# sebrahimi1988/dss-ml-at-scale

Measured on AMD Instinct MI355X. Metric: samples/sec, higher is better.
Workload: dtype bf16; 1 GPU; model=resnet18, global_batch=212, parallelism=dp1+hipgraph

## Files before the change

mi355x_scale/ops/csrc/bindings.cpp:

```cpp

#include <torch/extension.h>
#include <ATen/hip/HIPContext.h>
#include <hip/hip_runtime.h>

extern "C" void launch_normalize_u8_to_bf16(
    const uint8_t* in, void* out, const float* scale_dev,
    const float* shift_dev, long long n, hipStream_t stream);

void normalize_u8_to_bf16(torch::Tensor in, torch::Tensor out,
                          torch::Tensor scale, torch::Tensor shift) {
  TORCH_CHECK(in.is_cuda() && out.is_cuda(), "tensors must be on GPU");
  TORCH_CHECK(in.scalar_type() == torch::kUInt8, "input must be uint8");
  TORCH_CHECK(out.scalar_type() == torch::kBFloat16, "output must be bf16");
  TORCH_CHECK(in.is_contiguous(), "input must be contiguous (NHWC)");
  TORCH_CHECK(in.numel() == out.numel(), "element count mismatch");
  TORCH_CHECK(scale.is_cuda() && shift.is_cuda() && scale.numel() == 3 &&
                  shift.numel() == 3,
              "scale/shift must be 3-element device float tensors");
  TORCH_CHECK(scale.scalar_type() == torch::kFloat32 &&
              shift.scalar_type() == torch::kFloat32,
              "scale/shift must be float32");
  auto stream = at::cuda::getCurrentHIPStream();
  launch_normalize_u8_to_bf16(
      in.data_ptr<uint8_t>(), out.data_ptr(),
// ... 107 lines not shown
}

void diff_center(torch::Tensor yT, torch::Tensor wc, torch::Tensor wm,
                 int64_t S, int64_t d) {
  _check_f32(yT, "yT"); _check_f32(wc, "wc"); _check_f32(wm, "wm");
  auto stream = at::cuda::getCurrentHIPStream();
  launch_diff_center(yT.data_ptr<float>(), wc.data_ptr<float>(),
                     wm.data_ptr<float>(), yT.size(0), yT.size(1),
                     (int)S, (int)d, stream.stream());
}

void exog_project_mfma(torch::Tensor P, torch::Tensor wc,
                       torch::Tensor beta) {
  _check_f32(P, "P"); _check_f32(wc, "wc"); _check_f32(beta, "beta");
  TORCH_CHECK(P.size(1) == wc.size(0), "K mismatch");
  TORCH_CHECK(beta.size(0) == P.size(0) && beta.size(1) == wc.size(1));
  TORCH_CHECK(P.size(0) <= 16, "KX must fit one MFMA row tile");
  auto stream = at::cuda::getCurrentHIPStream();
  launch_exog_project_mfma(P.data_ptr<float>(), wc.data_ptr<float>(),
                           beta.data_ptr<float>(), P.size(1), wc.size(1),
                           P.size(0), stream.stream());
}


extern "C" int bn_reduce_blocks(long long rows, int C);
extern "C" void launch_bn_fwd_reduce(const void* x, float* partial,
                                     int nblocks, long long rows, int C,
                                     hipStream_t stream);
extern "C" void launch_bn_fwd_finalize(const float* partial, int nblocks,
                                       float* mean, float* invstd,
                                       float* running_mean,
                                       float* running_var, float momentum,
                                       float eps, long long rows, int C,
                                       int update_running, hipStream_t stream);
extern "C" void launch_bn_fwd_apply(const void* x, const void* res, void* y,
                                    const float* mean, const float* invstd,
                                    const float* weight, const float* bias,
                                    long long rows, int C, int relu,
                                    hipStream_t stream);
extern "C" void launch_bn_bwd_reduce(const void* dz, const void* y,
                                     const void* x, const float* mean,
                                     const float* invstd, float* partial,
                                     void* dym, int nblocks, long long rows,
                                     int C, int relu, hipStream_t stream);
extern "C" void launch_bn_bwd_reduce_rm(const void* dz, const void* x,
                                        const float* mean,
                                        const float* invstd,
                                        const float* weight,
                                        const float* bias, float* partial,
                                        void* dym, int nblocks,
                                        long long rows, int C,
                                        hipStream_t stream);
extern "C" void launch_bn_bwd_apply_rm(const void* dz, const void* x,
                                       const float* mean,
                                       const float* invstd,
                                       const float* bias, const float* k,
                                       void* dx, long long rows, int C,
                                       hipStream_t stream);
extern "C" void launch_bn_bwd_apply_dym(const void* dym, const void* x,
                                        const float* mean,
                                        const float* invstd, const float* k,
                                        void* dx, long long rows, int C,
                                        hipStream_t stream);
extern "C" void launch_bn_bwd_finalize(const float* partial, int nblocks,
                                       const float* invstd,
                                       const float* weight, float* dweight,
                                       float* dbias, float* k, long long rows,
// ... 2 lines not shown
extern "C" void launch_bn_bwd_apply(const void* dz, const void* y,
                                    const void* x, const float* mean,
                                    const float* invstd, const float* k,
                                    void* dx, void* dres, long long rows,
                                    int C, int relu, hipStream_t stream);

static void _check_bn_act(const torch::Tensor& t, const char* name) {
  TORCH_CHECK(t.is_cuda() && t.scalar_type() == torch::kBFloat16,
              name, " must be bf16 on GPU");
}

static long long _bn_rows(const torch::Tensor& x, int64_t C) {
  TORCH_CHECK(C % 8 == 0 && 256 % (C / 8) == 0,
              "C must be 8*2^k and <= 2048, got ", C);
  TORCH_CHECK(x.numel() % C == 0, "numel not divisible by C");
  return (long long)(x.numel() / C);
}

torch::Tensor bn_fwd_reduce(torch::Tensor x, int64_t C) {
  _check_bn_act(x, "x");
  long long rows = _bn_rows(x, C);
  int nb = bn_reduce_blocks(rows, (int)C);
  auto partial = torch::empty(
      {(int64_t)nb * 2 * C},
      torch::TensorOptions().dtype(torch::kFloat32).device(x.device()));
  launch_bn_fwd_reduce(x.data_ptr(), partial.data_ptr<float>(), nb, rows,
                       (int)C, at::cuda::getCurrentHIPStream().stream());
  return partial;
}

void bn_fwd_finalize(torch::Tensor partial, torch::Tensor mean,
                     torch::Tensor invstd, torch::Tensor running_mean,
                     torch::Tensor running_var, double momentum, double eps,
                     int64_t rows, int64_t C, bool update_running) {
  _check_f32(partial, "partial"); _check_f32(mean, "mean");
  _check_f32(invstd, "invstd");
  _check_f32(running_mean, "running_mean");
  _check_f32(running_var, "running_var");
  TORCH_CHECK(partial.numel() % (2 * C) == 0, "partial must be [nb*2C]");
  int nb = (int)(partial.numel() / (2 * C));
  launch_bn_fwd_finalize(partial.data_ptr<float>(), nb,
                         mean.data_ptr<float>(), invstd.data_ptr<float>(),
                         running_mean.data_ptr<float>(),
                         running_var.data_ptr<float>(), (float)momentum,
                         (float)eps, rows, (int)C, update_running ? 1 : 0,
                         at::cuda::getCurrentHIPStream().stream());
}

void bn_fwd_apply(torch::Tensor x, torch::Tensor res, torch::Tensor y,
                  torch::Tensor mean, torch::Tensor invstd,
                  torch::Tensor weight, torch::Tensor bias, int64_t C,
                  bool relu) {
  _check_bn_act(x, "x"); _check_bn_act(y, "y");
  _check_f32(mean, "mean"); _check_f32(invstd, "invstd");
  _check_f32(weight, "weight"); _check_f32(bias, "bias");
  const void* res_p = nullptr;
  if (res.defined() && res.numel()) {
    _check_bn_act(res, "res");
    TORCH_CHECK(res.numel() == x.numel(), "residual shape mismatch");
    res_p = res.data_ptr();
  }
  launch_bn_fwd_apply(x.data_ptr(), res_p, y.data_ptr(),
                      mean.data_ptr<float>(), invstd.data_ptr<float>(),
                      weight.data_ptr<float>(), bias.data_ptr<float>(),
                      _bn_rows(x, C), (int)C, relu ? 1 : 0,
                      at::cuda::getCurrentHIPStream().stream());
}

torch::Tensor bn_bwd_reduce(torch::Tensor dz, torch::Tensor y,
                            torch::Tensor x, torch::Tensor mean,
                            torch::Tensor invstd, torch::Tensor dym,
                            int64_t C, bool relu) {
  _check_bn_act(dz, "dz"); _check_bn_act(y, "y"); _check_bn_act(x, "x");
  void* dym_p = nullptr;
  if (dym.defined() && dym.numel()) {
    _check_bn_act(dym, "dym");
    TORCH_CHECK(dym.numel() == x.numel(), "dym shape mismatch");
    dym_p = dym.data_ptr();
  }
// ... 154 lines not shown
}

void bn_maxpool3x3s2_fwd(torch::Tensor x, torch::Tensor mean,
                         torch::Tensor invstd, torch::Tensor weight,
                         torch::Tensor bias, torch::Tensor y,
                         torch::Tensor code) {
  _check_bn_act(x, "x"); _check_bn_act(y, "y");
  _check_f32(mean, "mean"); _check_f32(invstd, "invstd");
  _check_f32(weight, "weight"); _check_f32(bias, "bias");
  TORCH_CHECK(code.scalar_type() == torch::kUInt8 && code.is_cuda());
  int N = x.size(0), C = x.size(1), H = x.size(2), W = x.size(3);
  int Ho = y.size(2), Wo = y.size(3);
  TORCH_CHECK(C % 8 == 0 && 256 % (C / 8) == 0, "bad C");
  TORCH_CHECK(Ho == (H + 1) / 2 && Wo == (W + 1) / 2, "3x3 s2 p1 shape");
  TORCH_CHECK(code.numel() == y.numel());
  launch_bn_maxpool_fwd(x.data_ptr(), mean.data_ptr<float>(),
                        invstd.data_ptr<float>(),
                        weight.data_ptr<float>(), bias.data_ptr<float>(),
                        y.data_ptr(), code.data_ptr<uint8_t>(),
                        N, H, W, Ho, Wo, C,
                        at::cuda::getCurrentHIPStream().stream());
}

void maxpool3x3s2_bwd(torch::Tensor dy, torch::Tensor code,
                      torch::Tensor dx) {
  _check_bn_act(dy, "dy"); _check_bn_act(dx, "dx");
  TORCH_CHECK(code.scalar_type() == torch::kUInt8 && code.is_cuda());
  int N = dx.size(0), C = dx.size(1), H = dx.size(2), W = dx.size(3);
  int Ho = dy.size(2), Wo = dy.size(3);
  TORCH_CHECK(code.numel() == dy.numel());
  launch_maxpool_bwd(dy.data_ptr(), code.data_ptr<uint8_t>(),
                     dx.data_ptr(), N, H, W, Ho, Wo, C,
                     at::cuda::getCurrentHIPStream().stream());
}

extern "C" void launch_adam_step(float* p, const float* g, float* m,
                                 float* v, int* step, float lr, float beta1,
                                 float beta2, float eps, float weight_decay,
                                 long long n, hipStream_t stream);

void adam_step(torch::Tensor p, torch::Tensor g, torch::Tensor m,
               torch::Tensor v, torch::Tensor step, double lr, double beta1,
               double beta2, double eps, double weight_decay) {
  _check_f32(p, "p"); _check_f32(g, "g"); _check_f32(m, "m");
  _check_f32(v, "v");
  TORCH_CHECK(step.is_cuda() && step.scalar_type() == torch::kInt32 &&
                  step.numel() == 1,
              "step must be a 1-element int32 device tensor");
  long long n = p.numel();
  TORCH_CHECK(g.numel() == n && m.numel() == n && v.numel() == n,
              "flat buffer length mismatch");
  launch_adam_step(p.data_ptr<float>(), g.data_ptr<float>(),
                   m.data_ptr<float>(), v.data_ptr<float>(),
                   step.data_ptr<int>(), (float)lr, (float)beta1,
                   (float)beta2, (float)eps, (float)weight_decay, n,
                   at::cuda::getCurrentHIPStream().stream());
}

extern "C" void launch_adam_step_mixed(float* master, const void* gb,
                                       const float* gf, float* m, float* v,
                                       void* pb, int* step, float lr,
                                       float beta1, float beta2, float eps,
                                       float weight_decay, long long nb,
                                       long long n, hipStream_t stream);

void adam_step_mixed(torch::Tensor master, torch::Tensor gb,
// ... 79 lines not shown

int64_t conv3x3_wrw_nchunks(int64_t Nb, int64_t H, int64_t C,
                            int64_t chunks) {
  return conv3x3_wrw_chunks((int)Nb, (int)H, (int)C, (int)chunks);
}

PYBIND11_MODULE(TORCH_EXTENSION_NAME, m) {
  m.def("conv3x3_wrw", &conv3x3_wrw,
        "MFMA 3x3/s1 CxC weight grad (fp32 accum, bf16 cast to view)",
        pybind11::arg("x"), pybind11::arg("dy"), pybind11::arg("part"),
        pybind11::arg("dw"), pybind11::arg("phase_mask") = 7,
        pybind11::arg("chunks") = 0);
  m.def("conv3x3_wrw_nchunks", &conv3x3_wrw_nchunks,
        "partial-buffer chunk count the wrw launcher will use");
  m.def("stem_conv_fwd", &stem_conv_fwd,
        "MFMA stem conv fwd (7x7 s2, 3->64, NHWC bf16)",
        pybind11::arg("x"), pybind11::arg("w"), pybind11::arg("out"),
        pybind11::arg("wp_scratch"), pybind11::arg("phase_mask") = 7);
  m.def("stem_conv_wrw", &stem_conv_wrw,
        "MFMA stem conv weight-grad (fp32 accum + bf16 cast)",
        pybind11::arg("x"), pybind11::arg("dy"), pybind11::arg("dw_f32"),
        pybind11::arg("dw"), pybind11::arg("phase_mask") = 7);
  m.def("normalize_u8_to_bf16", &normalize_u8_to_bf16,
        "fused uint8 NHWC -> normalized bf16 (same memory order)");
  m.def("groupfit_eval", &groupfit_eval,
        "batched per-group ARIMAX candidate evaluation (validation MSE)");
  m.def("groupfit_final", &groupfit_final,
        "batched per-group final fit (fitted values + params)");
  m.def("diff_center", &diff_center,
        "difference + per-group centering of the time-major panel");
  m.def("exog_project_mfma", &exog_project_mfma,
        "design-matrix GEMM beta = P @ Wc on f32 MFMA");
  m.def("bn_fwd_reduce", &bn_fwd_reduce);
  m.def("bn_fwd_finalize", &bn_fwd_finalize);
  m.def("bn_fwd_apply", &bn_fwd_apply);
  m.def("bn_bwd_reduce", &bn_bwd_reduce);
  m.def("bn_bwd_reduce_rm", &bn_bwd_reduce_rm);
  m.def("bn_bwd_apply_rm", &bn_bwd_apply_rm);
  m.def("bn_bwd_finalize", &bn_bwd_finalize);
  m.def("bn_bwd_apply", &bn_bwd_apply);
  m.def("bn_bwd_apply_dym", &bn_bwd_apply_dym);
  m.def("adam_step", &adam_step,
        "fused flat Adam step (one kernel over p/g/m/v)");
  m.def("maxpool3x3s2_fwd", &maxpool3x3s2_fwd);
  m.def("bn_maxpool3x3s2_fwd", &bn_maxpool3x3s2_fwd);
  m.def("maxpool3x3s2_bwd", &maxpool3x3s2_bwd);
  m.def("adam_step_mixed", &adam_step_mixed,
        "fused flat Adam with bf16 params/grads + fp32 master");
  m.def("arma_generate", &arma_generate,
        "batched ARMA(p,q) sample paths, one group per lane");
}
```

mi355x_scale/ops/csrc/fused_bn.hip:

```cpp

#include <hip/hip_runtime.h>
#include <hip/hip_bf16.h>

typedef __hip_bfloat16 bf16;

#define VEC 8

union BVec {
  uint4 u;
  bf16 h[VEC];
};

static __device__ __forceinline__ BVec load8(const bf16* p) {
  BVec v;
  v.u = *reinterpret_cast<const uint4*>(p);
  return v;
}

static __device__ __forceinline__ void store8(bf16* p, const BVec& v) {
  *reinterpret_cast<uint4*>(p) = v.u;
}

__global__ __launch_bounds__(256) void bn_fwd_reduce_kernel(
    const bf16* __restrict__ x, float* __restrict__ partial,
// ... 16 lines not shown
    }
  }

  __shared__ float lds[256 * 2 * VEC];
  float* mys = &lds[(rsub * lanes + lane) * 2 * VEC];
#pragma unroll
  for (int j = 0; j < VEC; ++j) {
    mys[j] = s[j];
    mys[VEC + j] = q[j];
  }
  __syncthreads();
  for (int step = rows_per_iter >> 1; step > 0; step >>= 1) {
    if (rsub < step) {
      const float* other = &lds[((rsub + step) * lanes + lane) * 2 * VEC];
#pragma unroll
      for (int j = 0; j < 2 * VEC; ++j) mys[j] += other[j];
    }
    __syncthreads();
  }
  if (rsub == 0) {
#pragma unroll
    for (int j = 0; j < VEC; ++j) {
      partial[(long long)(lane * VEC + j) * gridDim.x + blockIdx.x] = mys[j];
      partial[(long long)(C + lane * VEC + j) * gridDim.x + blockIdx.x] =
          mys[VEC + j];
    }
  }
}

__global__ __launch_bounds__(256) void bn_fwd_finalize_kernel(
    const float* __restrict__ partial, int nblocks,
    float* __restrict__ mean, float* __restrict__ invstd,
    float* __restrict__ running_mean, float* __restrict__ running_var,
    float momentum, float eps, long long rows, int C, int update_running) {
  int c = blockIdx.x * (blockDim.x / 64) + threadIdx.x / 64;
  int lane = threadIdx.x % 64;
  if (c >= C) return;
  float s = 0.f, q = 0.f;
  for (int b = lane; b < nblocks; b += 64) {
    s += partial[(long long)c * nblocks + b];
    q += partial[(long long)(C + c) * nblocks + b];
  }
#pragma unroll
  for (int off = 32; off > 0; off >>= 1) {
    s += __shfl_down(s, off, 64);
    q += __shfl_down(q, off, 64);
  }
  if (lane != 0) return;
  float n = (float)rows;
  float m = s / n;
  float var = fmaxf(q / n - m * m, 0.f);
  mean[c] = m;
  invstd[c] = rsqrtf(var + eps);
  if (update_running) {
    float unbiased = rows > 1 ? var * (n / (n - 1.f)) : var;
    running_mean[c] = (1.f - momentum) * running_mean[c] + momentum * m;
    running_var[c] = (1.f - momentum) * running_var[c] + momentum * unbiased;
  }
}

template <bool RELU, bool RES>
__global__ __launch_bounds__(256) void bn_fwd_apply_kernel(
    const bf16* __restrict__ x, const bf16* __restrict__ res,
    bf16* __restrict__ y, const float* __restrict__ mean,
    const float* __restrict__ invstd, const float* __restrict__ weight,
    const float* __restrict__ bias, long long rows, int C) {
  const int lanes = C / VEC;
  const int lane = threadIdx.x % lanes;
  const int rsub = threadIdx.x / lanes;
  const int rows_per_iter = blockDim.x / lanes;
  const long long rstride = (long long)gridDim.x * rows_per_iter;

  float a[VEC], b[VEC];
#pragma unroll
  for (int j = 0; j < VEC; ++j) {
    int c = lane * VEC + j;
    a[j] = weight[c] * invstd[c];
    b[j] = bias[c] - mean[c] * a[j];
  }

  for (long long row = (long long)blockIdx.x * rows_per_iter + rsub;
       row < rows; row += rstride) {
    const long long off = row * C + (long long)lane * VEC;
    BVec v = load8(x + off);
    BVec r;
    if (RES) r = load8(res + off);
    BVec o;
#pragma unroll
    for (int j = 0; j < VEC; ++j) {
      float f = fmaf(__bfloat162float(v.h[j]), a[j], b[j]);
      if (RES) f += __bfloat162float(r.h[j]);
// ... 150 lines not shown
  float m[VEC], is[VEC], wv[VEC], k1[VEC], k2[VEC];
#pragma unroll
  for (int j = 0; j < VEC; ++j) {
    int c = lane * VEC + j;
    m[j] = mean[c];
    is[j] = invstd[c];
    wv[j] = k[c];
    k1[j] = k[C + c];
    k2[j] = k[2 * C + c];
  }

  for (long long row = (long long)blockIdx.x * rows_per_iter + rsub;
       row < rows; row += rstride) {
    const long long off = row * C + (long long)lane * VEC;
    BVec g = load8(dz + off);
    BVec xv = load8(x + off);
    BVec yv;
    if (RELU) yv = load8(y + off);
    BVec odx, odr;
#pragma unroll
    for (int j = 0; j < VEC; ++j) {
      float dy = __bfloat162float(g.h[j]);
      if (RELU && __bfloat162float(yv.h[j]) <= 0.f) dy = 0.f;
      float xhat = (__bfloat162float(xv.h[j]) - m[j]) * is[j];
      float v = wv[j] * (dy - k1[j] - xhat * k2[j]);
      odx.h[j] = __float2bfloat16(v);
      if (RES) odr.h[j] = __float2bfloat16(dy);
    }
    store8(dx + off, odx);
    if (RES) store8(dres + off, odr);
  }
}

template <bool WRITE_DY>
__global__ __launch_bounds__(256) void bn_bwd_reduce_rm_kernel(
    const bf16* __restrict__ dz, const bf16* __restrict__ x,
    const float* __restrict__ mean, const float* __restrict__ invstd,
    const float* __restrict__ weight, const float* __restrict__ bias,
    float* __restrict__ partial, bf16* __restrict__ dym,
    long long rows, int C) {
  const int lanes = C / VEC;
  const int lane = threadIdx.x % lanes;
  const int rsub = threadIdx.x / lanes;
  const int rows_per_iter = blockDim.x / lanes;
  const long long rstride = (long long)gridDim.x * rows_per_iter;

  float m[VEC], is[VEC], wv[VEC], bv[VEC];
#pragma unroll
  for (int j = 0; j < VEC; ++j) {
    int c = lane * VEC + j;
    m[j] = mean[c];
    is[j] = invstd[c];
    wv[j] = weight[c];
    bv[j] = bias[c];
  }

  float sdy[VEC] = {0.f}, sdyx[VEC] = {0.f};
  for (long long row = (long long)blockIdx.x * rows_per_iter + rsub;
       row < rows; row += rstride) {
    const long long off = row * C + (long long)lane * VEC;
    BVec g = load8(dz + off);
    BVec xv = load8(x + off);
    BVec dyv;
#pragma unroll
    for (int j = 0; j < VEC; ++j) {
      float xhat = (__bfloat162float(xv.h[j]) - m[j]) * is[j];
      float dy = __bfloat162float(g.h[j]);
      if (wv[j] * xhat + bv[j] <= 0.f) dy = 0.f;
      sdy[j] += dy;
      sdyx[j] += dy * xhat;
      if (WRITE_DY) dyv.h[j] = __float2bfloat16(dy);
    }
    if (WRITE_DY) store8(dym + off, dyv);
  }

  __shared__ float lds[256 * 2 * VEC];
  float* mys = &lds[(rsub * lanes + lane) * 2 * VEC];
#pragma unroll
  for (int j = 0; j < VEC; ++j) {
    mys[j] = sdy[j];
    mys[VEC + j] = sdyx[j];
  }
  __syncthreads();
  for (int step = rows_per_iter >> 1; step > 0; step >>= 1) {
    if (rsub < step) {
      const float* other = &lds[((rsub + step) * lanes + lane) * 2 * VEC];
#pragma unroll
      for (int j = 0; j < 2 * VEC; ++j) mys[j] += other[j];
    }
    __syncthreads();
  }
  if (rsub == 0) {
#pragma unroll
    for (int j = 0; j < VEC; ++j) {
      partial[(long long)(lane * VEC + j) * gridDim.x + blockIdx.x] = mys[j];
      partial[(long long)(C + lane * VEC + j) * gridDim.x + blockIdx.x] =
          mys[VEC + j];
    }
  }
}

__global__ __launch_bounds__(256) void bn_bwd_apply_rm_kernel(
    const bf16* __restrict__ dz, const bf16* __restrict__ x,
    const float* __restrict__ mean, const float* __restrict__ invstd,
    const float* __restrict__ bias, const float* __restrict__ k,
    bf16* __restrict__ dx, long long rows, int C) {
  const int lanes = C / VEC;
  const int lane = threadIdx.x % lanes;
  const int rsub = threadIdx.x / lanes;
  const int rows_per_iter = blockDim.x / lanes;
  const long long rstride = (long long)gridDim.x * rows_per_iter;

  float m[VEC], is[VEC], wis[VEC], k1[VEC], k2[VEC], bv[VEC], wv[VEC];
#pragma unroll
  for (int j = 0; j < VEC; ++j) {
    int c = lane * VEC + j;
    m[j] = mean[c];
    is[j] = invstd[c];
    wis[j] = k[c];
    k1[j] = k[C + c];
    k2[j] = k[2 * C + c];
    bv[j] = bias[c];
    wv[j] = wis[j] / is[j];
  }

  for (long long row = (long long)blockIdx.x * rows_per_iter + rsub;
       row < rows; row += rstride) {
    const long long off = row * C + (long long)lane * VEC;
    BVec g = load8(dz + off);
    BVec xv = load8(x + off);
    BVec odx;
#pragma unroll
    for (int j = 0; j < VEC; ++j) {
      float xhat = (__bfloat162float(xv.h[j]) - m[j]) * is[j];
      float dy = __bfloat162float(g.h[j]);
      if (wv[j] * xhat + bv[j] <= 0.f) dy = 0.f;
      float v = wis[j] * (dy - k1[j] - xhat * k2[j]);
      odx.h[j] = __float2bfloat16(v);
    }
    store8(dx + off, odx);
  }
}


static int pick_grid(long long rows, int C) {
  int rows_per_iter = 256 / (C / VEC);
  long long blocks = (rows + rows_per_iter - 1) / rows_per_iter;
  if (blocks > 2080) blocks = 2080;
  return (int)(blocks > 0 ? blocks : 1);
}

extern "C" int bn_reduce_blocks(long long rows, int C) {
  int rows_per_iter = 256 / (C / VEC);
  long long blocks = (rows + rows_per_iter - 1) / rows_per_iter;
  if (blocks > 512) blocks = 512;
  return (int)(blocks > 0 ? blocks : 1);
}

extern "C" void launch_bn_fwd_reduce(const void* x, float* partial,
                                     int nblocks, long long rows, int C,
                                     hipStream_t stream) {
  hipLaunchKernelGGL(bn_fwd_reduce_kernel, dim3(nblocks), dim3(256), 0,
                     stream, (const bf16*)x, partial, rows, C);
}

extern "C" void launch_bn_fwd_finalize(const float* partial, int nblocks,
                                       float* mean, float* invstd,
                                       float* running_mean,
                                       float* running_var, float momentum,
                                       float eps, long long rows, int C,
                                       int update_running,
                                       hipStream_t stream) {
  hipLaunchKernelGGL(bn_fwd_finalize_kernel, dim3((C + 3) / 4),
                     dim3(256), 0, stream, partial, nblocks, mean, invstd,
                     running_mean, running_var, momentum, eps, rows, C,
                     update_running);
}

extern "C" void launch_bn_fwd_apply(const void* x, const void* res, void* y,
                                    const float* mean, const float* invstd,
                                    const float* weight, const float* bias,
                                    long long rows, int C, int relu,
                                    hipStream_t stream) {
  dim3 grid(pick_grid(rows, C)), block(256);
#define APPLY(R, S)                                                       \
  hipLaunchKernelGGL((bn_fwd_apply_kernel<R, S>), grid, block, 0, stream, \
                     (const bf16*)x, (const bf16*)res, (bf16*)y, mean,    \
                     invstd, weight, bias, rows, C)
  if (relu && res) APPLY(true, true);
  else if (relu) APPLY(true, false);
  else if (res) APPLY(false, true);
  else APPLY(false, false);
#undef APPLY
}

extern "C" void launch_bn_bwd_reduce(const void* dz, const void* y,
                                     const void* x, const float* mean,
                                     const float* invstd, float* partial,
                                     void* dym, int nblocks, long long rows,
                                     int C, int relu, hipStream_t stream) {
  dim3 grid(nblocks), block(256);
#define REDUCE(R, W)                                                       \
  hipLaunchKernelGGL((bn_bwd_reduce_kernel<R, W>), grid, block, 0, stream, \
                     (const bf16*)dz, (const bf16*)y, (const bf16*)x,      \
                     mean, invstd, partial, (bf16*)dym, rows, C)
  if (relu && dym) REDUCE(true, true);
  else if (relu) REDUCE(true, false);
  else if (dym) REDUCE(false, true);
  else REDUCE(false, false);
// ... 1 lines not shown
}

extern "C" void launch_bn_bwd_reduce_rm(const void* dz, const void* x,
                                        const float* mean,
                                        const float* invstd,
                                        const float* weight,
                                        const float* bias, float* partial,
                                        void* dym, int nblocks,
                                        long long rows, int C,
                                        hipStream_t stream) {
  dim3 grid(nblocks), block(256);
  if (dym)
    hipLaunchKernelGGL((bn_bwd_reduce_rm_kernel<true>), grid, block, 0,
                       stream, (const bf16*)dz, (const bf16*)x, mean,
                       invstd, weight, bias, partial, (bf16*)dym, rows, C);
  else
    hipLaunchKernelGGL((bn_bwd_reduce_rm_kernel<false>), grid, block, 0,
                       stream, (const bf16*)dz, (const bf16*)x, mean,
                       invstd, weight, bias, partial, nullptr, rows, C);
}

extern "C" void launch_bn_bwd_apply_rm(const void* dz, const void* x,
                                       const float* mean,
                                       const float* invstd,
                                       const float* bias, const float* k,
                                       void* dx, long long rows, int C,
                                       hipStream_t stream) {
  hipLaunchKernelGGL(bn_bwd_apply_rm_kernel, dim3(pick_grid(rows, C)),
                     dim3(256), 0, stream, (const bf16*)dz,
                     (const bf16*)x, mean, invstd, bias, k, (bf16*)dx,
                     rows, C);
}

extern "C" void launch_bn_bwd_apply_dym(const void* dym, const void* x,
                                        const float* mean,
                                        const float* invstd, const float* k,
                                        void* dx, long long rows, int C,
                                        hipStream_t stream) {
  hipLaunchKernelGGL(bn_bwd_apply_dym_kernel, dim3(pick_grid(rows, C)),
                     dim3(256), 0, stream, (const bf16*)dym, (const bf16*)x,
                     mean, invstd, k, (bf16*)dx, rows, C);
}

extern "C" void launch_bn_bwd_finalize(const float* partial, int nblocks,
                                       const float* invstd,
                                       const float* weight, float* dweight,
                                       float* dbias, float* k, long long rows,
                                       int C, int accumulate,
                                       hipStream_t stream) {
  hipLaunchKernelGGL(bn_bwd_finalize_kernel, dim3((C + 3) / 4),
                     dim3(256), 0, stream, partial, nblocks, invstd, weight,
                     dweight, dbias, k, rows, C, accumulate);
}

extern "C" void launch_bn_bwd_apply(const void* dz, const void* y,
                                    const void* x, const float* mean,
                                    const float* invstd, const float* k,
                                    void* dx, void* dres, long long rows,
                                    int C, int relu, hipStream_t stream) {
  dim3 grid(pick_grid(rows, C)), block(256);
#define APPLY(R, S)                                                        \
  hipLaunchKernelGGL((bn_bwd_apply_kernel<R, S>), grid, block, 0, stream,  \
                     (const bf16*)dz, (const bf16*)y, (const bf16*)x,      \
                     mean, invstd, k, (bf16*)dx, (bf16*)dres, rows, C)
  if (relu && dres) APPLY(true, true);
  else if (relu) APPLY(true, false);
// ... 5 lines not shown
```

mi355x_scale/ops/fused_bn.py:

```python
from __future__ import annotations

from typing import Optional

import torch
import torch.nn as nn
import torch.nn.functional as F

from . import _C, require_ext


def _hip_supported(x: torch.Tensor) -> bool:
    c = x.shape[1]
    return (x.is_cuda and x.dtype == torch.bfloat16 and x.dim() == 4
            and c % 8 == 0 and c <= 2048 and (256 % (c // 8)) == 0)


class _FusedBNFn(torch.autograd.Function):
    @staticmethod
    def forward(ctx, x, residual, weight, bias, running_mean, running_var,
                momentum, eps, relu):
        C = x.shape[1]
        rows = x.numel() // C
        dev = x.device
        mean = torch.empty(C, dtype=torch.float32, device=dev)
        invstd = torch.empty(C, dtype=torch.float32, device=dev)
        partial = _C.bn_fwd_reduce(x, C)
        _C.bn_fwd_finalize(partial, mean, invstd, running_mean, running_var,
                           momentum, eps, rows, C, True)
        y = torch.empty_like(x)
        res = residual if residual is not None else x.new_empty(0)
        _C.bn_fwd_apply(x, res, y, mean, invstd, weight, bias, C, relu)
        ctx.save_for_backward(x, y if residual is not None else x,
                              mean, invstd, weight, bias)
        ctx.relu = relu
        ctx.has_res = residual is not None
        return y

    @staticmethod
    def backward(ctx, dz):
        x, y, mean, invstd, weight, bias = ctx.saved_tensors
        C = x.shape[1]
        rows = x.numel() // C
        dev = x.device
        if not dz.is_contiguous(memory_format=torch.channels_last):
            dz = dz.contiguous(memory_format=torch.channels_last)
        k = torch.empty(3 * C, dtype=torch.float32, device=dev)
        def _grad_view(p):
            g = p.grad
            if (g is not None and g.is_cuda and g.is_contiguous()
                    and g.dtype == torch.float32 and g.numel() == C):
                return g
            return None

        import os
        wg, bg = _grad_view(weight), _grad_view(bias)
        fuse_acc = (torch.cuda.is_current_stream_capturing()
                    and wg is not None and bg is not None
                    and os.environ.get("MI355X_BN_FUSED_ACC", "1") == "1")
        if fuse_acc:
            dweight, dbias = wg, bg
        else:
            dweight = torch.empty(C, dtype=torch.float32, device=dev)
            dbias = torch.empty(C, dtype=torch.float32, device=dev)
        dx = torch.empty_like(x)
        if ctx.has_res:
            dym = torch.empty_like(x)
            partial = _C.bn_bwd_reduce(dz, y, x, mean, invstd, dym, C,
                                       ctx.relu)
            _C.bn_bwd_finalize(partial, invstd, weight, dweight, dbias, k,
                               rows, C, fuse_acc)
            _C.bn_bwd_apply_dym(dym, x, mean, invstd, k, dx, C)
            return (dx, dym, None if fuse_acc else dweight,
                    None if fuse_acc else dbias, None, None, None, None,
                    None)
        if ctx.relu:
            partial = _C.bn_bwd_reduce_rm(dz, x, mean, invstd, weight,
                                          bias, x.new_empty(0), C)
            _C.bn_bwd_finalize(partial, invstd, weight, dweight, dbias, k,
                               rows, C, fuse_acc)
            _C.bn_bwd_apply_rm(dz, x, mean, invstd, bias, k, dx, C)
        else:
            partial = _C.bn_bwd_reduce(dz, y, x, mean, invstd,
                                       x.new_empty(0), C, False)
            _C.bn_bwd_finalize(partial, invstd, weight, dweight, dbias, k,
                               rows, C, fuse_acc)
            _C.bn_bwd_apply(dz, y, x, mean, invstd, k, dx, x.new_empty(0),
                            C, False)
        return (dx, None, None if fuse_acc else dweight,
                None if fuse_acc else dbias, None, None, None, None, None)


class _FusedBNPoolFn(torch.autograd.Function):

    @staticmethod
    def forward(ctx, x, weight, bias, running_mean, running_var,
                momentum, eps, training):
        C = x.shape[1]
        dev = x.device
        if training:
            rows = x.numel() // C
            mean = torch.empty(C, dtype=torch.float32, device=dev)
            invstd = torch.empty(C, dtype=torch.float32, device=dev)
            partial = _C.bn_fwd_reduce(x, C)
            _C.bn_fwd_finalize(partial, mean, invstd, running_mean,
                               running_var, momentum, eps, rows, C, True)
        else:
            mean = running_mean.to(torch.float32)
            invstd = torch.rsqrt(running_var.to(torch.float32) + eps)
        n, _, h, w = x.shape
        ho, wo = (h + 1) // 2, (w + 1) // 2
        y = torch.empty((n, C, ho, wo), dtype=x.dtype, device=dev,
                        memory_format=torch.channels_last)
        code = torch.empty(n * ho * wo * C, dtype=torch.uint8, device=dev)
        _C.bn_maxpool3x3s2_fwd(x, mean, invstd, weight, bias, y, code)
        ctx.save_for_backward(x, mean, invstd, weight, bias, code)
        return y

    @staticmethod
    def backward(ctx, dp):
        x, mean, invstd, weight, bias, code = ctx.saved_tensors
        C = x.shape[1]
        rows = x.numel() // C
        dev = x.device
        if not dp.is_contiguous(memory_format=torch.channels_last):
            dp = dp.contiguous(memory_format=torch.channels_last)
        dz = torch.empty_like(x)
        _C.maxpool3x3s2_bwd(dp, code, dz)
        k = torch.empty(3 * C, dtype=torch.float32, device=dev)

        def _grad_view(p):
            g = p.grad
            if (g is not None and g.is_cuda and g.is_contiguous()
                    and g.dtype == torch.float32 and g.numel() == C):
                return g
            return None

        import os
        wg, bg = _grad_view(weight), _grad_view(bias)
        fuse_acc = (torch.cuda.is_current_stream_capturing()
                    and wg is not None and bg is not None
                    and os.environ.get("MI355X_BN_FUSED_ACC", "1") == "1")
        if fuse_acc:
            dweight, dbias = wg, bg
        else:
            dweight = torch.empty(C, dtype=torch.float32, device=dev)
            dbias = torch.empty(C, dtype=torch.float32, device=dev)
        dx = torch.empty_like(x)
        partial = _C.bn_bwd_reduce_rm(dz, x, mean, invstd, weight, bias,
                                      x.new_empty(0), C)
        _C.bn_bwd_finalize(partial, invstd, weight, dweight, dbias, k,
                           rows, C, fuse_acc)
        _C.bn_bwd_apply_rm(dz, x, mean, invstd, bias, k, dx, C)
        return (dx, None if fuse_acc else dweight,
                None if fuse_acc else dbias, None, None, None, None, None)


class FusedBNReLU2d(nn.Module):

    gpu_fallbacks: list = []

    def __init__(self, num_features: int, eps: float = 1e-5,
                 momentum: float = 0.1, relu: bool = True):
        super().__init__()
        self.num_features = num_features
        self.eps = eps
        self.momentum = momentum
        self.relu = relu
        self.weight = nn.Parameter(torch.ones(num_features))
        self.bias = nn.Parameter(torch.zeros(num_features))
        self.register_buffer("running_mean", torch.zeros(num_features))
        self.register_buffer("running_var", torch.ones(num_features))
        self.register_buffer("num_batches_tracked",
                             torch.tensor(0, dtype=torch.long))

    def extra_repr(self) -> str:
        return (f"{self.num_features}, eps={self.eps}, "
                f"momentum={self.momentum}, relu={self.relu}")

    def forward_pooled(self, x: torch.Tensor) -> torch.Tensor:
        assert self.relu, "pooled fusion is relu-only"
        if _hip_supported(x):
            require_ext()
            if self.training:
                self.num_batches_tracked += 1
            x = x.contiguous(memory_format=torch.channels_last)
            return _FusedBNPoolFn.apply(
                x, self.weight, self.bias, self.running_mean,
                self.running_var, self.momentum, self.eps, self.training)
        return F.max_pool2d(self.forward(x), 3, stride=2, padding=1)

    def forward(self, x: torch.Tensor,
                residual: Optional[torch.Tensor] = None) -> torch.Tensor:
        if self.training:
            self.num_batches_tracked += 1
        if _hip_supported(x):
            require_ext()
            x = x.contiguous(memory_format=torch.channels_last)
            if residual is not None:
                residual = residual.contiguous(
                    memory_format=torch.channels_last)
            if self.training:
                return _FusedBNFn.apply(
                    x, residual, self.weight, self.bias, self.running_mean,
                    self.running_var, self.momentum, self.eps, self.relu)
            if not (torch.is_grad_enabled() and
                    (x.requires_grad or self.weight.requires_grad)):
                invstd = torch.rsqrt(self.running_var + self.eps)
                y = torch.empty_like(x)
                res = (residual if residual is not None else x.new_empty(0))
                _C.bn_fwd_apply(x, res, y, self.running_mean, invstd,
                                self.weight, self.bias, x.shape[1],
                                self.relu)
                return y
        if x.is_cuda and len(FusedBNReLU2d.gpu_fallbacks) < 256:
            FusedBNReLU2d.gpu_fallbacks.append(
                (tuple(x.shape), str(x.dtype), self.training))
        y = F.batch_norm(x, self.running_mean, self.running_var, self.weight,
                         self.bias, self.training, self.momentum, self.eps)
        if residual is not None:
            y = y + residual
        return F.relu(y) if self.relu else y
```

Before: 25880 samples/s.

## Fuse max-unpool into stem BN backward and fold step counter into finalize

The stem BN+maxpool backward now rebuilds the max-unpool gradient in registers inside the BN reduce and apply kernels, so the full-resolution dz tensor is never written or read and the separate maxpool backward kernel goes away. Each BN layer's num_batches_tracked increment also moves into the finalize kernel, which removes one small add kernel per BN layer per step. The cost is that the unpool work runs twice, once in reduce and once in apply, and each output tile does extra gathers of dp and code. The old path stays available behind an environment flag.

Measured after the change: 26500 samples/s, median of 6. 1.02x the previous value.

```diff
diff --git a/mi355x_scale/ops/csrc/bindings.cpp b/mi355x_scale/ops/csrc/bindings.cpp
--- a/mi355x_scale/ops/csrc/bindings.cpp
+++ b/mi355x_scale/ops/csrc/bindings.cpp
@@ -163,7 +163,19 @@
                                        float* running_mean,
                                        float* running_var, float momentum,
                                        float eps, long long rows, int C,
-                                       int update_running, hipStream_t stream);
+                                       int update_running,
+                                       long long* num_batches_tracked,
+                                       hipStream_t stream);
+extern "C" void launch_bn_pool_bwd_reduce(
+    const void* dp, const unsigned char* code, const void* x,
+    const float* mean, const float* invstd, const float* weight,
+    const float* bias, float* partial, int nblocks, int N, int H, int W,
+    int Ho, int Wo, int C, hipStream_t stream);
+extern "C" void launch_bn_pool_bwd_apply(
+    const void* dp, const unsigned char* code, const void* x,
+    const float* mean, const float* invstd, const float* bias,
+    const float* k, void* dx, int N, int H, int W, int Ho, int Wo, int C,
+    hipStream_t stream);
 extern "C" void launch_bn_fwd_apply(const void* x, const void* res, void* y,
                                     const float* mean, const float* invstd,
                                     const float* weight, const float* bias,
@@ -232,19 +244,28 @@
 void bn_fwd_finalize(torch::Tensor partial, torch::Tensor mean,
                      torch::Tensor invstd, torch::Tensor running_mean,
                      torch::Tensor running_var, double momentum, double eps,
-                     int64_t rows, int64_t C, bool update_running) {
+                     int64_t rows, int64_t C, bool update_running,
+                     c10::optional<torch::Tensor> num_batches_tracked) {
   _check_f32(partial, "partial"); _check_f32(mean, "mean");
   _check_f32(invstd, "invstd");
   _check_f32(running_mean, "running_mean");
   _check_f32(running_var, "running_var");
   TORCH_CHECK(partial.numel() % (2 * C) == 0, "partial must be [nb*2C]");
   int nb = (int)(partial.numel() / (2 * C));
+  long long* nbt_p = nullptr;
+  if (num_batches_tracked.has_value()) {
+    const torch::Tensor& nbt = *num_batches_tracked;
+    TORCH_CHECK(nbt.is_cuda() && nbt.scalar_type() == torch::kInt64 &&
+                    nbt.numel() == 1,
+                "num_batches_tracked must be a 1-element int64 GPU tensor");
+    nbt_p = reinterpret_cast<long long*>(nbt.data_ptr<int64_t>());
+  }
   launch_bn_fwd_finalize(partial.data_ptr<float>(), nb,
                          mean.data_ptr<float>(), invstd.data_ptr<float>(),
                          running_mean.data_ptr<float>(),
                          running_var.data_ptr<float>(), (float)momentum,
                          (float)eps, rows, (int)C, update_running ? 1 : 0,
-                         at::cuda::getCurrentHIPStream().stream());
+                         nbt_p, at::cuda::getCurrentHIPStream().stream());
 }
 
 void bn_fwd_apply(torch::Tensor x, torch::Tensor res, torch::Tensor y,
@@ -465,6 +486,78 @@
   launch_maxpool_bwd(dy.data_ptr(), code.data_ptr<uint8_t>(),
                      dx.data_ptr(), N, H, W, Ho, Wo, C,
                      at::cuda::getCurrentHIPStream().stream());
+}
+
+struct _PoolGeom { int N, C, H, W, Ho, Wo; };
+
+static _PoolGeom _check_bn_pool_bwd(const torch::Tensor& dp,
+                                    const torch::Tensor& code,
+                                    const torch::Tensor& x) {
+  _check_bn_act(dp, "dp"); _check_bn_act(x, "x");
+  TORCH_CHECK(code.scalar_type() == torch::kUInt8 && code.is_cuda() &&
+                  code.is_contiguous(),
+              "code must be contiguous u8 on GPU");
+  TORCH_CHECK(x.dim() == 4 && dp.dim() == 4, "x and dp must be 4-d");
+  TORCH_CHECK(x.is_contiguous(at::MemoryFormat::ChannelsLast) &&
+                  dp.is_contiguous(at::MemoryFormat::ChannelsLast),
+              "x and dp must be channels_last");
+  _PoolGeom g{(int)x.size(0), (int)x.size(1), (int)x.size(2),
+              (int)x.size(3), (int)dp.size(2), (int)dp.size(3)};
+  TORCH_CHECK(g.C % 8 == 0 && 256 % (g.C / 8) == 0, "bad C");
+  TORCH_CHECK(dp.size(0) == g.N && dp.size(1) == g.C, "dp N/C mismatch");
+  TORCH_CHECK(g.Ho == (g.H + 1) / 2 && g.Wo == (g.W + 1) / 2,
+              "3x3 s2 p1 shape");
+  TORCH_CHECK(code.numel() == dp.numel(), "code/dp size mismatch");
+  TORCH_CHECK((int64_t)g.N * g.Ho * g.Wo < (int64_t(1) << 31),
+              "N*Ho*Wo must be < 2^31");
+  return g;
+}
+
+torch::Tensor bn_pool_bwd_reduce(torch::Tensor dp, torch::Tensor code,
+                                 torch::Tensor x, torch::Tensor mean,
+                                 torch::Tensor invstd, torch::Tensor weight,
+                                 torch::Tensor bias) {
+  _PoolGeom g = _check_bn_pool_bwd(dp, code, x);
+  _check_f32(mean, "mean"); _check_f32(invstd, "invstd");
+  _check_f32(weight, "weight"); _check_f32(bias, "bias");
+  TORCH_CHECK(mean.numel() == g.C && invstd.numel() == g.C &&
+                  weight.numel() == g.C && bias.numel() == g.C,
+              "channel vectors must be [C]");
+  int nb = bn_reduce_blocks((long long)g.N * g.Ho * g.Wo, g.C);
+  auto partial = torch::empty(
+      {(int64_t)nb * 2 * g.C},
+      torch::TensorOptions().dtype(torch::kFloat32).device(x.device()));
+  launch_bn_pool_bwd_reduce(dp.data_ptr(), code.data_ptr<uint8_t>(),
+                            x.data_ptr(), mean.data_ptr<float>(),
+                            invstd.data_ptr<float>(),
+                            weight.data_ptr<float>(),
+                            bias.data_ptr<float>(),
+                            partial.data_ptr<float>(), nb, g.N, g.H, g.W,
+                            g.Ho, g.Wo, g.C,
+                            at::cuda::getCurrentHIPStream().stream());
+  return partial;
+}
+
+void bn_pool_bwd_apply(torch::Tensor dp, torch::Tensor code, torch::Tensor x,
+                       torch::Tensor mean, torch::Tensor invstd,
+                       torch::Tensor bias, torch::Tensor k,
+                       torch::Tensor dx) {
+  _PoolGeom g = _check_bn_pool_bwd(dp, code, x);
+  _check_bn_act(dx, "dx");
+  _check_f32(mean, "mean"); _check_f32(invstd, "invstd");
+  _check_f32(bias, "bias"); _check_f32(k, "k");
+  TORCH_CHECK(mean.numel() == g.C && invstd.numel() == g.C &&
+                  bias.numel() == g.C && k.numel() == 3 * g.C,
+              "channel vectors must be [C], k [3C]");
+  TORCH_CHECK(dx.sizes() == x.sizes() &&
+                  dx.is_contiguous(at::MemoryFormat::ChannelsLast),
+              "dx must match x (channels_last)");
+  launch_bn_pool_bwd_apply(dp.data_ptr(), code.data_ptr<uint8_t>(),
+                           x.data_ptr(), mean.data_ptr<float>(),
+                           invstd.data_ptr<float>(), bias.data_ptr<float>(),
+                           k.data_ptr<float>(), dx.data_ptr(), g.N, g.H,
+                           g.W, g.Ho, g.Wo, g.C,
+                           at::cuda::getCurrentHIPStream().stream());
 }
 
 extern "C" void launch_adam_step(float* p, const float* g, float* m,
@@ -610,7 +703,14 @@
   m.def("exog_project_mfma", &exog_project_mfma,
         "design-matrix GEMM beta = P @ Wc on f32 MFMA");
   m.def("bn_fwd_reduce", &bn_fwd_reduce);
-  m.def("bn_fwd_finalize", &bn_fwd_finalize);
+  m.def("bn_fwd_finalize", &bn_fwd_finalize,
+        "mean/invstd + running stats (+ optional int64 step counter)",
+        pybind11::arg("partial"), pybind11::arg("mean"),
+        pybind11::arg("invstd"), pybind11::arg("running_mean"),
+        pybind11::arg("running_var"), pybind11::arg("momentum"),
+        pybind11::arg("eps"), pybind11::arg("rows"), pybind11::arg("C"),
+        pybind11::arg("update_running"),
+        pybind11::arg("num_batches_tracked") = pybind11::none());
   m.def("bn_fwd_apply", &bn_fwd_apply);
   m.def("bn_bwd_reduce", &bn_bwd_reduce);
   m.def("bn_bwd_reduce_rm", &bn_bwd_reduce_rm);
@@ -623,6 +723,10 @@
   m.def("maxpool3x3s2_fwd", &maxpool3x3s2_fwd);
   m.def("bn_maxpool3x3s2_fwd", &bn_maxpool3x3s2_fwd);
   m.def("maxpool3x3s2_bwd", &maxpool3x3s2_bwd);
+  m.def("bn_pool_bwd_reduce", &bn_pool_bwd_reduce,
+        "stem BN bwd reduce with the max-unpool rebuilt in registers");
+  m.def("bn_pool_bwd_apply", &bn_pool_bwd_apply,
+        "stem BN bwd apply with the max-unpool rebuilt in registers");
   m.def("adam_step_mixed", &adam_step_mixed,
         "fused flat Adam with bf16 params/grads + fp32 master");
   m.def("arma_generate", &arma_generate,
diff --git a/mi355x_scale/ops/csrc/fused_bn.hip b/mi355x_scale/ops/csrc/fused_bn.hip
--- a/mi355x_scale/ops/csrc/fused_bn.hip
+++ b/mi355x_scale/ops/csrc/fused_bn.hip
@@ -72,7 +72,8 @@
     const float* __restrict__ partial, int nblocks,
     float* __restrict__ mean, float* __restrict__ invstd,
     float* __restrict__ running_mean, float* __restrict__ running_var,
-    float momentum, float eps, long long rows, int C, int update_running) {
+    float momentum, float eps, long long rows, int C, int update_running,
+    long long* __restrict__ num_batches_tracked) {
   int c = blockIdx.x * (blockDim.x / 64) + threadIdx.x / 64;
   int lane = threadIdx.x % 64;
   if (c >= C) return;
@@ -97,6 +98,7 @@
     running_mean[c] = (1.f - momentum) * running_mean[c] + momentum * m;
     running_var[c] = (1.f - momentum) * running_var[c] + momentum * unbiased;
   }
+  if (c == 0 && num_batches_tracked) *num_batches_tracked += 1;
 }
 
 template <bool RELU, bool RES>
@@ -313,6 +315,24 @@
   }
 }
 
+static __device__ __forceinline__ float rm_masked_dy(float dy, float w,
+                                                     float xhat, float b) {
+  if (fmaf(w, xhat, b) <= 0.f) dy = 0.f;
+  return dy;
+}
+
+static __device__ __forceinline__ void rm_accumulate(float dy, float xhat,
+                                                     float& sdy,
+                                                     float& sdyx) {
+  sdy += dy;
+  sdyx = fmaf(dy, xhat, sdyx);
+}
+
+static __device__ __forceinline__ float rm_dx(float wis, float dy, float k1,
+                                              float xhat, float k2) {
+  return wis * fmaf(-xhat, k2, dy - k1);
+}
+
 template <bool WRITE_DY>
 __global__ __launch_bounds__(256) void bn_bwd_reduce_rm_kernel(
     const bf16* __restrict__ dz, const bf16* __restrict__ x,
@@ -346,10 +366,8 @@
 #pragma unroll
     for (int j = 0; j < VEC; ++j) {
       float xhat = (__bfloat162float(xv.h[j]) - m[j]) * is[j];
-      float dy = __bfloat162float(g.h[j]);
-      if (wv[j] * xhat + bv[j] <= 0.f) dy = 0.f;
-      sdy[j] += dy;
-      sdyx[j] += dy * xhat;
+      float dy = rm_masked_dy(__bfloat162float(g.h[j]), wv[j], xhat, bv[j]);
+      rm_accumulate(dy, xhat, sdy[j], sdyx[j]);
       if (WRITE_DY) dyv.h[j] = __float2bfloat16(dy);
     }
     if (WRITE_DY) store8(dym + off, dyv);
@@ -414,12 +432,199 @@
 #pragma unroll
     for (int j = 0; j < VEC; ++j) {
       float xhat = (__bfloat162float(xv.h[j]) - m[j]) * is[j];
-      float dy = __bfloat162float(g.h[j]);
-      if (wv[j] * xhat + bv[j] <= 0.f) dy = 0.f;
-      float v = wis[j] * (dy - k1[j] - xhat * k2[j]);
+      float dy = rm_masked_dy(__bfloat162float(g.h[j]), wv[j], xhat, bv[j]);
+      float v = rm_dx(wis[j], dy, k1[j], xhat, k2[j]);
       odx.h[j] = __float2bfloat16(v);
     }
     store8(dx + off, odx);
+  }
+}
+
+union CVec {
+  uint2 u;
+  unsigned char c[VEC];
+};
+
+struct PoolTile {
+  float a[4][VEC];
+  long long pix[4];
+  bool valid[4];
+};
+
+static __device__ __forceinline__ void unpool_tile(
+    const bf16* __restrict__ dp, const unsigned char* __restrict__ code,
+    int r32, int lane, int H, int W, int Ho, int Wo, int C, PoolTile& t) {
+  const int j = r32 % Wo;
+  const int t32 = r32 / Wo;
+  const int i = t32 % Ho;
+  const int n = t32 / Ho;
+  const long long lvec = (long long)lane * VEC;
+
+  BVec g00{}, g01{}, g10{}, g11{};
+  CVec c00{}, c01{}, c10{}, c11{};
+  const bool v01 = (j + 1 < Wo), v10 = (i + 1 < Ho);
+  const long long base = (((long long)n * Ho + i) * Wo + j) * C + lvec;
+  g00.u = *reinterpret_cast<const uint4*>(dp + base);
+  c00.u = *reinterpret_cast<const uint2*>(code + base);
+  if (v01) {
+    g01.u = *reinterpret_cast<const uint4*>(dp + base + C);
+    c01.u = *reinterpret_cast<const uint2*>(code + base + C);
+  }
+  if (v10) {
+    const long long b2 = base + (long long)Wo * C;
+    g10.u = *reinterpret_cast<const uint4*>(dp + b2);
+    c10.u = *reinterpret_cast<const uint2*>(code + b2);
+    if (v01) {
+      g11.u = *reinterpret_cast<const uint4*>(dp + b2 + C);
+      c11.u = *reinterpret_cast<const uint2*>(code + b2 + C);
+    }
+  }
+#pragma unroll
+  for (int k = 0; k < VEC; ++k) {
+    float a00 = (c00.c[k] == 4) ? __bfloat162float(g00.h[k]) : 0.f;
+    float a01 = (c00.c[k] == 5) ? __bfloat162float(g00.h[k]) : 0.f;
+    if (v01 && c01.c[k] == 3) a01 += __bfloat162float(g01.h[k]);
+    float a10 = (c00.c[k] == 7) ? __bfloat162float(g00.h[k]) : 0.f;
+    if (v10 && c10.c[k] == 1) a10 += __bfloat162float(g10.h[k]);
+    float a11 = (c00.c[k] == 8) ? __bfloat162float(g00.h[k]) : 0.f;
+    if (v01 && c01.c[k] == 6) a11 += __bfloat162float(g01.h[k]);
+    if (v10 && c10.c[k] == 2) a11 += __bfloat162float(g10.h[k]);
+    if (v10 && v01 && c11.c[k] == 0) a11 += __bfloat162float(g11.h[k]);
+    t.a[0][k] = __bfloat162float(__float2bfloat16(a00));
+    t.a[1][k] = __bfloat162float(__float2bfloat16(a01));
+    t.a[2][k] = __bfloat162float(__float2bfloat16(a10));
+    t.a[3][k] = __bfloat162float(__float2bfloat16(a11));
+  }
+  const int h0 = 2 * i, w0 = 2 * j;
+  const bool r1 = (h0 + 1 < H), cL1 = (w0 + 1 < W);
+  const long long ibase = (((long long)n * H + h0) * W + w0) * C + lvec;
+  t.pix[0] = ibase;
+  t.pix[1] = ibase + C;
+  t.pix[2] = ibase + (long long)W * C;
+  t.pix[3] = ibase + (long long)W * C + C;
+  t.valid[0] = true;
+  t.valid[1] = cL1;
+  t.valid[2] = r1;
+  t.valid[3] = r1 && cL1;
+}
+
+__global__ __launch_bounds__(256) void bn_pool_bwd_reduce_kernel(
+    const bf16* __restrict__ dp, const unsigned char* __restrict__ code,
+    const bf16* __restrict__ x, const float* __restrict__ mean,
+    const float* __restrict__ invstd, const float* __restrict__ weight,
+    const float* __restrict__ bias, float* __restrict__ partial, int N,
+    int H, int W, int Ho, int Wo, int C) {
+  const int lanes = C / VEC;
+  const int lane = threadIdx.x % lanes;
+  const int rsub = threadIdx.x / lanes;
+  const int rows_per_iter = blockDim.x / lanes;
+  const long long tiles = (long long)N * Ho * Wo;
+  const long long rstride = (long long)gridDim.x * rows_per_iter;
+
+  float m[VEC], is[VEC], wv[VEC], bv[VEC];
+#pragma unroll
+  for (int j = 0; j < VEC; ++j) {
+    int c = lane * VEC + j;
+    m[j] = mean[c];
+    is[j] = invstd[c];
+    wv[j] = weight[c];
+    bv[j] = bias[c];
+  }
+
+  float sdy[VEC] = {0.f}, sdyx[VEC] = {0.f};
+  for (long long row = (long long)blockIdx.x * rows_per_iter + rsub;
+       row < tiles; row += rstride) {
+    PoolTile t;
+    unpool_tile(dp, code, (int)row, lane, H, W, Ho, Wo, C, t);
+    BVec xv[4];
+#pragma unroll
+    for (int p = 0; p < 4; ++p)
+      if (t.valid[p]) xv[p] = load8(x + t.pix[p]);
+#pragma unroll
+    for (int p = 0; p < 4; ++p) {
+      if (!t.valid[p]) continue;
+#pragma unroll
+      for (int j = 0; j < VEC; ++j) {
+        float xhat = (__bfloat162float(xv[p].h[j]) - m[j]) * is[j];
+        float dy = rm_masked_dy(t.a[p][j], wv[j], xhat, bv[j]);
+        rm_accumulate(dy, xhat, sdy[j], sdyx[j]);
+      }
+    }
+  }
+
+  __shared__ float lds[256 * 2 * VEC];
+  float* mys = &lds[(rsub * lanes + lane) * 2 * VEC];
+#pragma unroll
+  for (int j = 0; j < VEC; ++j) {
+    mys[j] = sdy[j];
+    mys[VEC + j] = sdyx[j];
+  }
+  __syncthreads();
+  for (int step = rows_per_iter >> 1; step > 0; step >>= 1) {
+    if (rsub < step) {
+      const float* other = &lds[((rsub + step) * lanes + lane) * 2 * VEC];
+#pragma unroll
+      for (int j = 0; j < 2 * VEC; ++j) mys[j] += other[j];
+    }
+    __syncthreads();
+  }
+  if (rsub == 0) {
+#pragma unroll
+    for (int j = 0; j < VEC; ++j) {
+      partial[(long long)(lane * VEC + j) * gridDim.x + blockIdx.x] = mys[j];
+      partial[(long long)(C + lane * VEC + j) * gridDim.x + blockIdx.x] =
+          mys[VEC + j];
+    }
+  }
+}
+
+__global__ __launch_bounds__(256) void bn_pool_bwd_apply_kernel(
+    const bf16* __restrict__ dp, const unsigned char* __restrict__ code,
+    const bf16* __restrict__ x, const float* __restrict__ mean,
+    const float* __restrict__ invstd, const float* __restrict__ bias,
+    const float* __restrict__ k, bf16* __restrict__ dx, int N, int H, int W,
+    int Ho, int Wo, int C) {
+  const int lanes = C / VEC;
+  const int lane = threadIdx.x % lanes;
+  const int rsub = threadIdx.x / lanes;
+  const int rows_per_iter = blockDim.x / lanes;
+  const long long tiles = (long long)N * Ho * Wo;
+  const long long rstride = (long long)gridDim.x * rows_per_iter;
+
+  float m[VEC], is[VEC], wis[VEC], k1[VEC], k2[VEC], bv[VEC], wv[VEC];
+#pragma unroll
+  for (int j = 0; j < VEC; ++j) {
+    int c = lane * VEC + j;
+    m[j] = mean[c];
+    is[j] = invstd[c];
+    wis[j] = k[c];
+    k1[j] = k[C + c];
+    k2[j] = k[2 * C + c];
+    bv[j] = bias[c];
+    wv[j] = wis[j] / is[j];
+  }
+
+  for (long long row = (long long)blockIdx.x * rows_per_iter + rsub;
+       row < tiles; row += rstride) {
+    PoolTile t;
+    unpool_tile(dp, code, (int)row, lane, H, W, Ho, Wo, C, t);
+    BVec xv[4];
+#pragma unroll
+    for (int p = 0; p < 4; ++p)
+      if (t.valid[p]) xv[p] = load8(x + t.pix[p]);
+#pragma unroll
+    for (int p = 0; p < 4; ++p) {
+      if (!t.valid[p]) continue;
+      BVec odx;
+#pragma unroll
+      for (int j = 0; j < VEC; ++j) {
+        float xhat = (__bfloat162float(xv[p].h[j]) - m[j]) * is[j];
+        float dy = rm_masked_dy(t.a[p][j], wv[j], xhat, bv[j]);
+        float v = rm_dx(wis[j], dy, k1[j], xhat, k2[j]);
+        odx.h[j] = __float2bfloat16(v);
+      }
+      store8(dx + t.pix[p], odx);
+    }
   }
 }
 
@@ -451,11 +656,12 @@
                                        float* running_var, float momentum,
                                        float eps, long long rows, int C,
                                        int update_running,
+                                       long long* num_batches_tracked,
                                        hipStream_t stream) {
   hipLaunchKernelGGL(bn_fwd_finalize_kernel, dim3((C + 3) / 4),
                      dim3(256), 0, stream, partial, nblocks, mean, invstd,
                      running_mean, running_var, momentum, eps, rows, C,
-                     update_running);
+                     update_running, num_batches_tracked);
 }
 
 extern "C" void launch_bn_fwd_apply(const void* x, const void* res, void* y,
@@ -523,6 +729,27 @@
                      rows, C);
 }
 
+extern "C" void launch_bn_pool_bwd_reduce(
+    const void* dp, const unsigned char* code, const void* x,
+    const float* mean, const float* invstd, const float* weight,
+    const float* bias, float* partial, int nblocks, int N, int H, int W,
+    int Ho, int Wo, int C, hipStream_t stream) {
+  hipLaunchKernelGGL(bn_pool_bwd_reduce_kernel, dim3(nblocks), dim3(256), 0,
+                     stream, (const bf16*)dp, code, (const bf16*)x, mean,
+                     invstd, weight, bias, partial, N, H, W, Ho, Wo, C);
+}
+
+extern "C" void launch_bn_pool_bwd_apply(
+    const void* dp, const unsigned char* code, const void* x,
+    const float* mean, const float* invstd, const float* bias,
+    const float* k, void* dx, int N, int H, int W, int Ho, int Wo, int C,
+    hipStream_t stream) {
+  hipLaunchKernelGGL(bn_pool_bwd_apply_kernel,
+                     dim3(pick_grid((long long)N * Ho * Wo, C)), dim3(256),
+                     0, stream, (const bf16*)dp, code, (const bf16*)x, mean,
+                     invstd, bias, k, (bf16*)dx, N, H, W, Ho, Wo, C);
+}
+
 extern "C" void launch_bn_bwd_apply_dym(const void* dym, const void* x,
                                         const float* mean,
                                         const float* invstd, const float* k,
diff --git a/mi355x_scale/ops/fused_bn.py b/mi355x_scale/ops/fused_bn.py
--- a/mi355x_scale/ops/fused_bn.py
+++ b/mi355x_scale/ops/fused_bn.py
@@ -18,7 +18,7 @@
 class _FusedBNFn(torch.autograd.Function):
     @staticmethod
     def forward(ctx, x, residual, weight, bias, running_mean, running_var,
-                momentum, eps, relu):
+                momentum, eps, relu, num_batches_tracked):
         C = x.shape[1]
         rows = x.numel() // C
         dev = x.device
@@ -26,7 +26,7 @@
         invstd = torch.empty(C, dtype=torch.float32, device=dev)
         partial = _C.bn_fwd_reduce(x, C)
         _C.bn_fwd_finalize(partial, mean, invstd, running_mean, running_var,
-                           momentum, eps, rows, C, True)
+                           momentum, eps, rows, C, True, num_batches_tracked)
         y = torch.empty_like(x)
         res = residual if residual is not None else x.new_empty(0)
         _C.bn_fwd_apply(x, res, y, mean, invstd, weight, bias, C, relu)
@@ -72,7 +72,7 @@
             _C.bn_bwd_apply_dym(dym, x, mean, invstd, k, dx, C)
             return (dx, dym, None if fuse_acc else dweight,
                     None if fuse_acc else dbias, None, None, None, None,
-                    None)
+                    None, None)
         if ctx.relu:
             partial = _C.bn_bwd_reduce_rm(dz, x, mean, invstd, weight,
                                           bias, x.new_empty(0), C)
@@ -87,14 +87,15 @@
             _C.bn_bwd_apply(dz, y, x, mean, invstd, k, dx, x.new_empty(0),
                             C, False)
         return (dx, None, None if fuse_acc else dweight,
-                None if fuse_acc else dbias, None, None, None, None, None)
+                None if fuse_acc else dbias, None, None, None, None, None,
+                None)
 
 
 class _FusedBNPoolFn(torch.autograd.Function):
 
     @staticmethod
     def forward(ctx, x, weight, bias, running_mean, running_var,
-                momentum, eps, training):
+                momentum, eps, training, num_batches_tracked):
         C = x.shape[1]
         dev = x.device
         if training:
@@ -103,7 +104,8 @@
             invstd = torch.empty(C, dtype=torch.float32, device=dev)
             partial = _C.bn_fwd_reduce(x, C)
             _C.bn_fwd_finalize(partial, mean, invstd, running_mean,
-                               running_var, momentum, eps, rows, C, True)
+                               running_var, momentum, eps, rows, C, True,
+                               num_batches_tracked)
         else:
             mean = running_mean.to(torch.float32)
             invstd = torch.rsqrt(running_var.to(torch.float32) + eps)
@@ -124,8 +126,8 @@
         dev = x.device
         if not dp.is_contiguous(memory_format=torch.channels_last):
             dp = dp.contiguous(memory_format=torch.channels_last)
-        dz = torch.empty_like(x)
-        _C.maxpool3x3s2_bwd(dp, code, dz)
+        import os
+        fused_unpool = os.environ.get("MI355X_BN_POOL_FUSED_BWD", "1") != "0"
         k = torch.empty(3 * C, dtype=torch.float32, device=dev)
 
         def _grad_view(p):
@@ -135,7 +137,6 @@
                 return g
             return None
 
-        import os
         wg, bg = _grad_view(weight), _grad_view(bias)
         fuse_acc = (torch.cuda.is_current_stream_capturing()
                     and wg is not None and bg is not None
@@ -146,13 +147,23 @@
             dweight = torch.empty(C, dtype=torch.float32, device=dev)
             dbias = torch.empty(C, dtype=torch.float32, device=dev)
         dx = torch.empty_like(x)
-        partial = _C.bn_bwd_reduce_rm(dz, x, mean, invstd, weight, bias,
-                                      x.new_empty(0), C)
-        _C.bn_bwd_finalize(partial, invstd, weight, dweight, dbias, k,
-                           rows, C, fuse_acc)
-        _C.bn_bwd_apply_rm(dz, x, mean, invstd, bias, k, dx, C)
+        if fused_unpool:
+            partial = _C.bn_pool_bwd_reduce(dp, code, x, mean, invstd,
+                                            weight, bias)
+            _C.bn_bwd_finalize(partial, invstd, weight, dweight, dbias, k,
+                               rows, C, fuse_acc)
+            _C.bn_pool_bwd_apply(dp, code, x, mean, invstd, bias, k, dx)
+        else:
+            dz = torch.empty_like(x)
+            _C.maxpool3x3s2_bwd(dp, code, dz)
+            partial = _C.bn_bwd_reduce_rm(dz, x, mean, invstd, weight, bias,
+                                          x.new_empty(0), C)
+            _C.bn_bwd_finalize(partial, invstd, weight, dweight, dbias, k,
+                               rows, C, fuse_acc)
+            _C.bn_bwd_apply_rm(dz, x, mean, invstd, bias, k, dx, C)
         return (dx, None if fuse_acc else dweight,
-                None if fuse_acc else dbias, None, None, None, None, None)
+                None if fuse_acc else dbias, None, None, None, None, None,
+                None)
 
 
 class FusedBNReLU2d(nn.Module):
@@ -181,18 +192,15 @@
         assert self.relu, "pooled fusion is relu-only"
         if _hip_supported(x):
             require_ext()
-            if self.training:
-                self.num_batches_tracked += 1
             x = x.contiguous(memory_format=torch.channels_last)
             return _FusedBNPoolFn.apply(
                 x, self.weight, self.bias, self.running_mean,
-                self.running_var, self.momentum, self.eps, self.training)
+                self.running_var, self.momentum, self.eps, self.training,
+                self.num_batches_tracked)
         return F.max_pool2d(self.forward(x), 3, stride=2, padding=1)
 
     def forward(self, x: torch.Tensor,
                 residual: Optional[torch.Tensor] = None) -> torch.Tensor:
-        if self.training:
-            self.num_batches_tracked += 1
         if _hip_supported(x):
             require_ext()
             x = x.contiguous(memory_format=torch.channels_last)
@@ -202,7 +210,8 @@
             if self.training:
                 return _FusedBNFn.apply(
                     x, residual, self.weight, self.bias, self.running_mean,
-                    self.running_var, self.momentum, self.eps, self.relu)
+                    self.running_var, self.momentum, self.eps, self.relu,
+                    self.num_batches_tracked)
             if not (torch.is_grad_enabled() and
                     (x.requires_grad or self.weight.requires_grad)):
                 invstd = torch.rsqrt(self.running_var + self.eps)
@@ -212,6 +221,8 @@
                                 self.weight, self.bias, x.shape[1],
                                 self.relu)
                 return y
+        if self.training:
+            self.num_batches_tracked += 1
         if x.is_cuda and len(FusedBNReLU2d.gpu_fallbacks) < 256:
             FusedBNReLU2d.gpu_fallbacks.append(
                 (tuple(x.shape), str(x.dtype), self.training))
```
